# zhiqwang/demonet

Measured on AMD Instinct MI355X. Metric: images/sec ssdlite320_mobilenet_v3_large fp16 end-to-end incl. NMS, higher is better.
Workload: dtype fp16; 1 GPU; ssdlite320_mobilenet_v3_large fp16, batch 64 per GPU, 320x320 synthetic images, K=91, synthetic weights seed 0, post-process incl. per-class top-300 + hard NMS; global_batch=64, forwards_in_flight=3, parallelism=single GPU, input=NCHW fp32 in [0,1], device-resident

## Files before the change

### demonet_amd/_lib.py

```python
import ctypes as C
import os

_HERE = os.path.dirname(os.path.abspath(__file__))
LIB_PATH = os.environ.get("DEMONET_HIP_LIB") or os.path.join(_HERE, "lib", "libdemonet_hip.so")
DN_ABI_VERSION = 1

DN_OP = dict(stem=1, pw=2, dw=3, se=4, conv=5, maxpool=6, l2norm=7)
DN_T = dict(act=0, image=1, vec=2, pool=3)
DN_NMS = dict(hard=0, linear=1, gaussian=2)
DN_MERGE = dict(iou=0, ios=1)
DN_FRAME = dict(nv12=0, i420=1, rgb24=2, bgr24=3)
DN_COLOR = dict(bt601=0, bt709=1)
DN_COLOR_FULL_RANGE = 0x10
DN_REGION_HFLIP = 1
DN_SGD_CHUNK = 2048
DN_SGD_MAX_GATE = 8


class TensorDesc(C.Structure):
    _fields_ = [("c", C.c_int32), ("h", C.c_int32), ("w", C.c_int32), ("kind", C.c_int32)]


class OpDesc(C.Structure):
    _fields_ = [("type", C.c_int32), ("inp", C.c_int32), ("out", C.c_int32), ("residual", C.c_int32),
# ... 25 lines not shown

class TrackParams(C.Structure):
    _fields_ = [("track_thresh", C.c_float), ("low_thresh", C.c_float), ("new_thresh", C.c_float),
                ("match_thresh", C.c_float), ("second_thresh", C.c_float), ("unconfirmed_thresh", C.c_float),
                ("track_buffer", C.c_int32), ("class_agnostic", C.c_int32), ("max_tracks", C.c_int32), ("reserved", C.c_int32)]


class ModelDesc(C.Structure):
    _fields_ = [("abi_version", C.c_int32), ("n_tensors", C.c_int32), ("n_ops", C.c_int32),
                ("tensors", C.POINTER(TensorDesc)), ("ops", C.POINTER(OpDesc)),
                ("input_tensor", C.c_int32), ("image_h", C.c_int32), ("image_w", C.c_int32),
                ("mean", C.c_float * 3), ("std", C.c_float * 3),
                ("num_classes", C.c_int32), ("n_levels", C.c_int32),
                ("level_tensor", C.c_int32 * 8), ("anchors_per_loc", C.c_int32 * 8),
                ("num_anchors", C.c_int32), ("anchors", C.POINTER(C.c_float)),
                ("score_thresh", C.c_float), ("nms_thresh", C.c_float),
                ("detections_per_img", C.c_int32), ("topk_candidates", C.c_int32)]


_SIGNATURES = {
    "dn_abi_version": (C.c_int, []),
    "dn_last_error": (C.c_char_p, []),
    "dn_create": (C.c_int, [C.POINTER(ModelDesc), C.c_void_p, C.c_size_t, C.POINTER(C.c_void_p)]),
    "dn_destroy": (None, [C.c_void_p]),
    "dn_workspace_bytes": (C.c_size_t, [C.c_void_p, C.c_int]),
    "dn_forward": (C.c_int, [C.c_void_p, C.c_void_p, C.c_int, C.c_int, C.c_int, C.c_void_p, C.c_void_p, C.c_void_p,
                             C.c_void_p, C.c_void_p, C.c_size_t, C.c_void_p]),
    "dn_forward_u8": (C.c_int, [C.c_void_p, C.c_void_p, C.c_int, C.c_int, C.c_int, C.c_void_p, C.c_void_p, C.c_void_p,
                             C.c_void_p, C.c_void_p, C.c_size_t, C.c_void_p]),
    "dn_forward_frames": (C.c_int, [C.c_void_p, C.c_void_p, C.c_int, C.c_int, C.c_int, C.c_void_p, C.c_void_p, C.c_void_p,
                                    C.c_void_p, C.c_void_p, C.c_size_t, C.c_void_p]),
    "dn_forward_regions": (C.c_int, [C.c_void_p, C.c_void_p, C.c_void_p, C.c_int, C.c_int, C.c_int, C.c_void_p, C.c_void_p, C.c_void_p,
                                     C.c_void_p, C.c_void_p, C.c_size_t, C.c_void_p]),
    "dn_forward_heads": (C.c_int, [C.c_void_p, C.c_void_p, C.c_int, C.c_int, C.c_int, C.c_void_p, C.c_size_t, C.c_void_p]),
    "dn_head_outputs": (C.c_int, [C.c_void_p, C.c_void_p, C.c_int, C.POINTER(C.c_void_p), C.POINTER(C.c_void_p)]),
    "dn_tensor_ptr": (C.c_int, [C.c_void_p, C.c_void_p, C.c_int, C.c_int, C.POINTER(C.c_void_p), C.POINTER(C.c_size_t)]),
    "dn_postprocess_workspace_bytes": (C.c_size_t, [C.c_int, C.c_int, C.c_int, C.c_int, C.c_int]),
    "dn_postprocess": (C.c_int, [C.c_void_p, C.c_void_p, C.c_void_p, C.c_int, C.c_int, C.c_int, C.c_float, C.c_float,
                                 C.c_void_p, C.c_float, C.c_float, C.c_int, C.c_int, C.c_void_p, C.c_void_p, C.c_void_p,
                                 C.c_void_p, C.c_void_p, C.c_void_p, C.c_size_t, C.c_void_p]),
    "dn_postprocess_soft": (C.c_int, [C.c_void_p, C.c_void_p, C.c_void_p, C.c_int, C.c_int, C.c_int, C.c_float, C.c_float,
                                      C.c_void_p, C.c_float, C.c_float, C.c_int, C.c_float, C.c_int, C.c_int, C.c_void_p, C.c_void_p, C.c_void_p,
                                      C.c_void_p, C.c_void_p, C.c_void_p, C.c_size_t, C.c_void_p]),
    "dn_set_nms": (C.c_int, [C.c_void_p, C.c_int, C.c_float]),
    "dn_pointwise_conv": (C.c_int, [C.c_void_p, C.c_void_p, C.c_void_p, C.c_void_p, C.c_void_p, C.c_void_p, C.c_void_p, C.c_int,
                                    C.c_int, C.c_int, C.c_int, C.c_int, C.c_int, C.c_int64, C.c_void_p]),
    "dn_depthwise_conv": (C.c_int, [C.c_void_p, C.c_void_p, C.c_void_p, C.c_void_p, C.c_int, C.c_int, C.c_int, C.c_int,
                                    C.c_int, C.c_int, C.c_int, C.c_int, C.c_void_p]),
    "dn_depthwise_pool_blocks": (C.c_int, [C.c_int] * 6),
    "dn_depthwise_conv_pool": (C.c_int, [C.c_void_p] * 4 + [C.c_int] * 8 + [C.c_void_p] * 7 + [C.c_int, C.c_void_p]),
    "dn_dense_conv": (C.c_int, [C.c_void_p] * 5 + [C.c_int] * 10 + [C.c_void_p]),
    "dn_expand_depthwise": (C.c_int, [C.c_void_p] * 9 + [C.c_int] * 11 + [C.c_void_p]),
    "dn_expand_depthwise_tiles": (C.c_int, [C.c_int, C.c_int, C.c_int]),
    "dn_ssd_loss_workspace_bytes": (C.c_size_t, [C.c_int, C.c_int]),
    "dn_ssd_loss": (C.c_int, [C.c_void_p] * 6 + [C.c_int] * 4 + [C.c_float, C.c_float] + [C.c_void_p, C.c_void_p, C.c_void_p, C.c_size_t, C.c_void_p]),
    "dn_ssd_loss_state_bytes": (C.c_size_t, [C.c_int, C.c_int]),
    "dn_ssd_loss_train": (C.c_int, [C.c_void_p] * 6 + [C.c_int] * 4 + [C.c_float, C.c_float] + [C.c_void_p, C.c_void_p, C.c_void_p, C.c_size_t, C.c_void_p, C.c_size_t,
                                    C.c_void_p]),
    "dn_ssd_loss_backward": (C.c_int, [C.c_void_p] * 6 + [C.c_size_t, C.c_void_p] + [C.c_int] * 4 + [C.c_void_p] * 3),
    "dn_set_graph_mode": (C.c_int, [C.c_void_p, C.c_int]),
    "dn_set_packed_output": (C.c_int, [C.c_void_p, C.c_void_p]),
    "dn_profile_begin": (C.c_int, [C.c_void_p]),
    "dn_profile_end": (C.c_int, [C.c_void_p, C.POINTER(C.c_float), C.c_int]),
    "dn_batch_split": (C.c_int, [C.c_void_p, C.c_int]),
    "dn_set_chains": (C.c_int, [C.c_void_p, C.c_int]),
    "dn_profile_op_info": (C.c_int, [C.c_void_p, C.c_int, C.c_char_p, C.c_int, C.POINTER(C.c_int32)]),
    "dn_level_features": (C.c_int, [C.c_void_p, C.c_void_p, C.c_int, C.c_int, C.c_int, C.POINTER(C.c_void_p), C.POINTER(C.c_int), C.POINTER(C.c_int)]),
    "dn_forward_features": (C.c_int, [C.c_void_p, C.c_void_p, C.c_int, C.c_int, C.c_int, C.c_void_p, C.c_size_t, C.c_void_p]),
    "dn_lite_head_backward_workspace_bytes": (C.c_size_t, [C.c_int] * 6),
    "dn_lite_head_backward": (C.c_int, [C.c_void_p] * 5 + [C.c_int64] + [C.c_int] * 5 + [C.c_void_p] * 5 + [C.c_size_t, C.c_void_p]),
    "dn_crop_tiles": (C.c_int, [C.c_void_p, C.c_int, C.c_int, C.c_void_p, C.c_int, C.c_int, C.c_int, C.c_void_p, C.c_void_p]),
    "dn_merge_detections_workspace_bytes": (C.c_size_t, [C.c_int] * 3),
    "dn_merge_detections": (C.c_int, [C.c_void_p] * 5 + [C.c_int, C.c_int, C.POINTER(C.c_int32), C.c_int, C.c_int, C.c_float, C.c_int, C.c_int] + [C.c_void_p] * 6
                            + [C.c_size_t, C.c_void_p]),
    "dn_fuse_detections_workspace_bytes": (C.c_size_t, [C.c_int, C.c_int, C.POINTER(C.c_int32), C.c_int]),
    "dn_fuse_detections": (C.c_int, [C.c_void_p] * 6 + [C.c_int, C.c_int, C.POINTER(C.c_int32), C.c_int, C.c_float, C.c_float, C.c_int] + [C.c_void_p] * 6
                           + [C.c_size_t, C.c_void_p]),
    "dn_match_detections": (C.c_int, [C.c_void_p] * 8 + [C.c_int] * 4 + [C.POINTER(C.c_double), C.c_int, C.c_double] + [C.c_void_p] * 5),
    "dn_coco_match": (C.c_int, [C.c_void_p] * 9 + [C.c_int] * 4 + [C.POINTER(C.c_double), C.c_int, C.POINTER(C.c_double), C.c_int, C.c_int] + [C.c_void_p] * 5),
    "dn_augment_workspace_bytes": (C.c_size_t, [C.c_int]),
    "dn_augment_batch": (C.c_int, [C.POINTER(C.c_void_p), C.POINTER(C.c_int32), C.POINTER(C.c_int32), C.c_int, C.c_int, C.c_int, C.c_void_p, C.c_void_p, C.c_size_t, C.c_void_p]),
    "dn_sgd_workspace_bytes": (C.c_size_t, [C.c_int, C.c_int]),
    "dn_grad_norm": (C.c_int, [C.c_void_p, C.c_int, C.c_int, C.c_void_p, C.c_size_t, C.c_void_p, C.c_void_p]),
    "dn_sgd_step": (C.c_int, [C.c_void_p, C.c_int, C.c_int, SgdHyper, C.c_void_p, C.c_int, C.c_void_p, C.c_float, C.c_void_p, C.c_void_p]),
    "dn_track_state_bytes": (C.c_size_t, [C.c_int, C.c_int]),
    "dn_track_reset": (C.c_int, [C.c_void_p, C.c_int, C.c_int, C.c_void_p, C.c_void_p]),
    "dn_track_update": (C.c_int, [C.c_void_p] * 4 + [C.c_int, C.c_int, C.POINTER(TrackParams), C.c_void_p, C.c_size_t] + [C.c_void_p] * 8),
}
EXPORTS = tuple(_SIGNATURES)
_DEBUG_SIGNATURES = {
    "dn_debug_last_kernel": (C.c_int, [C.c_char_p, C.c_int]),
    "dn_debug_conv_pool": (C.c_int, [C.c_void_p] * 6 + [C.c_int] * 6 + [C.c_void_p]),
    "dn_debug_stem": (C.c_int, [C.c_void_p] * 4 + [C.c_int] * 7 + [C.POINTER(C.c_float), C.POINTER(C.c_float), C.c_int, C.c_int, C.c_void_p]),
    "dn_debug_choice": (C.c_int, [C.c_char_p, C.POINTER(C.c_int64), C.c_int, C.c_char_p, C.c_int]),
}

_lib = None


class HipLibraryMissing(RuntimeError):
    pass


def lib():
    global _lib
    if _lib is not None:
# ... 39 lines not shown
```

### demonet_amd/csrc/plan.hip

```cpp
#include <stdarg.h>
#include <stdlib.h>
#include <string.h>

#include <algorithm>
#include <cmath>
#include <atomic>
#include <map>
#include <mutex>
#include <set>
#include <string>
#include <tuple>
#include <vector>

#include "choice.h"

static thread_local char g_err[512] = "";

static thread_local char g_kernel[96] = "";
void dn_note_kernel(const char* fmt, ...) {
    va_list ap;
    va_start(ap, fmt);
    vsnprintf(g_kernel, sizeof(g_kernel), fmt, ap);
    va_end(ap);
}
// ... 1389 lines not shown
    a.nms_method = nms_method; a.nms_sigma = nms_sigma;
    a.boxes = boxes; a.scores = scores; a.labels = labels; a.counts = counts; a.kept_anchor = kept_anchor;
    a.ws = ws; a.ws_bytes = ws_bytes;
    a.xq = xcd_images_per_group(n);
    return launch_postprocess(a, reinterpret_cast<hipStream_t>(stream), nullptr);
}

extern "C" int dn_postprocess(const float* logits, const float* reg, const float* anchors, int n, int A, int K, float image_h,
                              float image_w, const float* scale_xy, float score_thresh, float nms_thresh, int topk, int dets,
                              float* boxes, float* scores, int64_t* labels, int32_t* counts, int32_t* kept_anchor, void* ws,
                              size_t ws_bytes, void* stream) {
    return dn_postprocess_soft(logits, reg, anchors, n, A, K, image_h, image_w, scale_xy, score_thresh, nms_thresh, DN_NMS_HARD, 0.f, topk, dets,
                               boxes, scores, labels, counts, kept_anchor, ws, ws_bytes, stream);
}

extern "C" int dn_pointwise_conv(const void* x, const void* w, const void* w_frag, const float* bias, const void* residual,
                                 const float* se, void* out, int m, int cin, int cout, int hw, int act, int out_fp32,
                                 int64_t out_img_stride, void* stream) {
    DN_REQUIRE(x && w && bias && out, "dn_pointwise_conv: null argument");
    PwArgs a;
    a.x = reinterpret_cast<const half_t*>(x); a.w = reinterpret_cast<const half_t*>(w); a.bias = bias;
    a.wfrag = reinterpret_cast<const half_t*>(w_frag);
    a.residual = reinterpret_cast<const half_t*>(residual); a.se = se; a.out = out;
    a.m = m; a.cin = cin; a.cout = cout; a.hw = hw; a.act = act; a.out_fp32 = out_fp32;
    a.out_img_stride = out_fp32 ? (long)out_img_stride : 0; a.out_base = 0;
    a.xq = (hw > 0 && m % hw == 0) ? xcd_images_per_group(m / hw) : 0;
    int rc = launch_pointwise(a, reinterpret_cast<hipStream_t>(stream));
    if (rc) return rc;
    DN_HIP_CHECK(hipGetLastError());
    return DN_OK;
}

extern "C" int dn_expand_depthwise(const void* x, const void* w1, const float* b1, const void* wd, const float* bd, const void* w3,
                                   const float* b3, void* out, float* pool_partial, int n, int h, int w, int cin, int cexp, int cout,
                                   int k, int stride, int act1, int act2, int has_res, void* stream) {
    DN_REQUIRE(x && wd && bd && out, "dn_expand_depthwise: null argument");
    DN_REQUIRE((w1 == nullptr) == (b1 == nullptr) && (w3 == nullptr) == (b3 == nullptr), "dn_expand_depthwise: weight without bias");
    ExpDwArgs a{};
    a.x = reinterpret_cast<const half_t*>(x); a.out = reinterpret_cast<half_t*>(out); a.pool = pool_partial;
    a.w1 = reinterpret_cast<const half_t*>(w1); a.b1 = b1; a.wd = reinterpret_cast<const half_t*>(wd); a.bd = bd;
    a.w3 = reinterpret_cast<const half_t*>(w3); a.b3 = b3;
    a.n = n; a.H = h; a.W = w; a.k = k; a.stride = stride; a.pad = (k - 1) / 2;
    a.Ho = (h + 2 * a.pad - k) / stride + 1; a.Wo = (w + 2 * a.pad - k) / stride + 1;
    a.cin = cin; a.cexp = cexp; a.cout = w3 ? cout : cexp; a.act1 = act1; a.act2 = act2; a.has_res = has_res;
    a.xq = xcd_images_per_group(n);
    int rc = launch_expdw(a, reinterpret_cast<hipStream_t>(stream));
    if (rc) return rc;
    DN_HIP_CHECK(hipGetLastError());
    return DN_OK;
}

extern "C" int dn_expand_depthwise_tiles(int ho, int wo, int stride) { return expdw_tiles_per_image(ho, wo, stride); }

extern "C" int dn_dense_conv(const void* x, const void* w, const float* bias, const void* zeros, void* out, int n, int h, int wd,
                             int cin, int cout, int k, int stride, int pad, int dil, int act, void* stream) {
    DN_REQUIRE(x && w && bias && out, "dn_dense_conv: null argument");
    DN_REQUIRE(n > 0 && h > 0 && wd > 0 && k >= 1 && stride >= 1 && dil >= 1 && pad >= 0, "dn_dense_conv: bad geometry");
    ConvArgs a;
    a.x = reinterpret_cast<const half_t*>(x); a.w = reinterpret_cast<const half_t*>(w); a.bias = bias; a.out = out;
    a.zeros = reinterpret_cast<const half_t*>(zeros);
    a.n = n; a.h = h; a.w_ = wd; a.cin = cin; a.cout = cout; a.k = k; a.stride = stride; a.pad = pad; a.dil = dil; a.act = act;
    a.ho = (h + 2 * pad - dil * (k - 1) - 1) / stride + 1;
    a.wo = (wd + 2 * pad - dil * (k - 1) - 1) / stride + 1;
    DN_REQUIRE(a.ho > 0 && a.wo > 0, "dn_dense_conv: empty output");
    a.out_fp32 = 0; a.out_img_stride = 0; a.out_base = 0;
    a.xq = xcd_images_per_group(n);
    int rc = launch_conv(a, reinterpret_cast<hipStream_t>(stream));
    if (rc) return rc;
    DN_HIP_CHECK(hipGetLastError());
    return DN_OK;
}

extern "C" int dn_depthwise_conv(const void* x, const void* w, const float* bias, void* out, int n, int h, int wd, int c, int k,
                                 int stride, int pad, int act, void* stream) {
    DN_REQUIRE(x && w && bias && out, "dn_depthwise_conv: null argument");
    DwArgs a;
    a.x = reinterpret_cast<const half_t*>(x); a.w = reinterpret_cast<const half_t*>(w); a.bias = bias;
    a.out = reinterpret_cast<half_t*>(out);
    a.n = n; a.h = h; a.w_ = wd; a.c = c; a.k = k; a.stride = stride; a.pad = pad; a.act = act;
    a.ho = (h + 2 * pad - k) / stride + 1;
    a.wo = (wd + 2 * pad - k) / stride + 1;
    a.xq = xcd_images_per_group(n);
    int rc = launch_depthwise(a, reinterpret_cast<hipStream_t>(stream));
    if (rc) return rc;
    DN_HIP_CHECK(hipGetLastError());
    return DN_OK;
}

extern "C" int dn_depthwise_pool_blocks(int h, int wd, int c, int k, int stride, int pad) {
    DwArgs a{};
    a.n = 1; a.h = h; a.w_ = wd; a.c = c; a.k = k; a.stride = stride; a.pad = pad;
    a.ho = (h + 2 * pad - k) / stride + 1;
    a.wo = (wd + 2 * pad - k) / stride + 1;
    return depthwise_pool_blocks(a);
}

extern "C" int dn_depthwise_conv_pool(const void* x, const void* w, const float* bias, void* out, int n, int h, int wd, int c, int k,
                                      int stride, int pad, int act, float* pool, const void* se_w1t, const float* se_b1, const void* se_w2t,
                                      const float* se_b2, float* se_scale, unsigned* se_counter, int squeeze, void* stream) {
    DN_REQUIRE(x && w && bias && out && pool, "dn_depthwise_conv_pool: null argument");
    DN_REQUIRE(!se_scale || (se_w1t && se_b1 && se_w2t && se_b2 && se_counter), "dn_depthwise_conv_pool: the squeeze-excitation tail needs both FCs and the counters");
    DwArgs a;
    a.x = reinterpret_cast<const half_t*>(x); a.w = reinterpret_cast<const half_t*>(w); a.bias = bias;
    a.out = reinterpret_cast<half_t*>(out);
    a.n = n; a.h = h; a.w_ = wd; a.c = c; a.k = k; a.stride = stride; a.pad = pad; a.act = act;
    a.ho = (h + 2 * pad - k) / stride + 1;
// ... 187 lines not shown
```

### demonet_amd/csrc/pwdirect.hip

```cpp
#include <algorithm>

#include "common.h"
#include "choice.h"

__device__ const uint4 g_pwdw_zero16 = {0u, 0u, 0u, 0u};

namespace {

typedef unsigned uint2v __attribute__((ext_vector_type(2)));

__device__ __forceinline__ void act16(floatx16& v, int act) {
    asm volatile("s_nop 7\n\ts_nop 3" : "+v"(v));
    if (act == DN_ACT_RELU) {
#pragma unroll
        for (int e = 0; e < 16; ++e) v[e] = dn_relu(v[e]);
    } else if (act == DN_ACT_RELU6) {
#pragma unroll
        for (int e = 0; e < 16; ++e) v[e] = dn_relu6(v[e]);
    } else if (act == DN_ACT_HSWISH) {
#pragma unroll
        for (int e = 0; e < 16; ++e) v[e] = v[e] * dn_relu6(v[e] + 3.f) * (1.f / 6.f);
    }
}

// ... 352 lines not shown
#pragma unroll
        for (int t = 0; t < 9; ++t) {
            const cp4 wp = (cp4)(q.wd + t * K + ks * 16);
            const u4v w0 = wp[0], w1 = wp[1];
            const uint4 wsel = make_uint4(hh ? w1[0] : w0[0], hh ? w1[1] : w0[1], hh ? w1[2] : w0[2], hh ? w1[3] : w0[3]);
            fma_mix_h8(acc, *reinterpret_cast<const uint4*>(&xin[t]), wsel);
        }
        dn_act_n<float[8], 8>(acc, q.act_dw);
#pragma unroll
        for (int e = 0; e < 8; ++e) xf[ks][e] = (half_t)acc[e];
    }
    const half8 zero8 = {0, 0, 0, 0, 0, 0, 0, 0};
    const half8 ones = {(half_t)1.f, (half_t)1.f, 0, 0, 0, 0, 0, 0};
    const half_t bhi = (half_t)bl;
    const half8 bw = {bhi, (half_t)(bl - (float)bhi), 0, 0, 0, 0, 0, 0};
    const bool bcol = kb == K;
    floatx16 acc;
#pragma unroll
    for (int e = 0; e < 16; ++e) acc[e] = 0.f;
#pragma unroll
    for (int ks = 0; ks < KSF; ++ks) acc = __builtin_amdgcn_mfma_f32_32x32x16_f16(wf[ks], xf[ks], acc, 0, 0, 0);
    acc = __builtin_amdgcn_mfma_f32_32x32x16_f16(bcol ? bw : zero8, bcol ? ones : zero8, acc, 0, 0, 0);
    act16(acc, a.act);
    if (has_res) {
#pragma unroll
        for (int g = 0; g < 4; ++g) {
            const half4 rr = __builtin_bit_cast(half4, rres[g]);
#pragma unroll
            for (int e = 0; e < 4; ++e) acc[4 * g + e] += (float)rr[e];
        }
    }
    uint2v p[4];
#pragma unroll
    for (int g = 0; g < 4; ++g) {
        half4 hv;
#pragma unroll
        for (int e = 0; e < 4; ++e) hv[e] = (half_t)acc[4 * g + e];
        p[g] = __builtin_bit_cast(uint2v, hv);
    }
    uint4 lo4, hi4;
    {
        const uint2v s0 = __builtin_amdgcn_permlane32_swap(p[0][0], p[1][0], false, false);
        const uint2v s1 = __builtin_amdgcn_permlane32_swap(p[0][1], p[1][1], false, false);
        const uint2v s2 = __builtin_amdgcn_permlane32_swap(p[2][0], p[3][0], false, false);
        const uint2v s3 = __builtin_amdgcn_permlane32_swap(p[2][1], p[3][1], false, false);
        lo4 = make_uint4(s0[0], s1[0], s0[1], s1[1]);
        hi4 = make_uint4(s2[0], s3[0], s2[1], s3[1]);
    }
    half_t* orow = reinterpret_cast<half_t*>(a.out) + (size_t)row * NC + hh * 8;
    const int c0 = hh * 8;
    if (row < mend) {
        if (c0 < NC) *reinterpret_cast<uint4*>(orow) = lo4;
        if (c0 + 16 < NC) *reinterpret_cast<uint4*>(orow + 16) = hi4;
    }
}


__device__ __forceinline__ void pw_glds16(const void* gsrc, unsigned dst) {
    unsigned keep;
    asm volatile("s_mov_b32 %0, m0\n\ts_mov_b32 m0, %2\n\ts_nop 0\n\tglobal_load_lds_dwordx4 %1, off\n\ts_mov_b32 m0, %0"
                 : "=&s"(keep) : "v"(gsrc), "s"(dst) : "memory");
}

template <int KS1, int RT>
__global__ __launch_bounds__(256) void pw_wstat_kernel(PwArgs a, int runs, int wg_per_group) {
    extern __shared__ __attribute__((aligned(16))) unsigned char pws_lds[];
    constexpr int KSF = KS1 - 1;
    typedef unsigned u32x4 __attribute__((ext_vector_type(4)));
    const int lane = threadIdx.x & 63, r = lane & 31, hh = lane >> 5;
    const int wave = __builtin_amdgcn_readfirstlane(threadIdx.x >> 6);
    const int K = a.cin, NC = a.cout;
    const int ksw = (K + 15) >> 4;
    int r0, mend, w;
    if (a.xq > 0) {
        const int g = blockIdx.x & 7;
        w = blockIdx.x >> 3;
        r0 = g * a.xq * a.hw;
        mend = min(a.m, r0 + a.xq * a.hw);
    } else {
        w = blockIdx.x; r0 = 0; mend = a.m;
    }
    const int run = w % runs, wgq = w / runs;
    const int Q = (wg_per_group / runs) * 4;
    const int n_units = mend > r0 ? (mend - r0 + 31) >> 5 : 0;
    const int ctiles = (NC + 31) >> 5;
    const int ct0 = run * RT;
    const unsigned lds0 = (unsigned)(size_t)(__attribute__((address_space(3))) unsigned char*)pws_lds;
    const unsigned xoff = (unsigned)(RT * ksw * 1024 + wave * ksw * 1024);
    auto dma_x = [&](int u) {
        const long row0 = (long)r0 + (long)u * 32;
        const unsigned char* src = reinterpret_cast<const unsigned char*>(a.x + row0 * K);
        const unsigned lim = (unsigned)min((long)(a.m - row0) * K * 2 - 16, 0x7fffffffL);
#pragma unroll 1
        for (int p = 0; p < ksw; ++p) pw_glds16(src + min((unsigned)(p * 1024 + lane * 16), lim), lds0 + xoff + p * 1024);
    };
    int u = wgq * 4 + wave;
    if (u < n_units) dma_x(u);
    {
        const unsigned char* wsrc = reinterpret_cast<const unsigned char*>(a.wfrag) + (size_t)ct0 * ksw * 1024 + lane * 16;
        const int pieces = max(min(RT, ctiles - ct0), 0) * ksw;
#pragma unroll 1
        for (int p = wave; p < pieces; p += 4) pw_glds16(wsrc + (size_t)p * 1024, lds0 + p * 1024);
    }
    float bl[RT];
#pragma unroll
    for (int t = 0; t < RT; ++t) bl[t] = a.bias[min((ct0 + t) * 32 + r, NC - 1)];
// ... 47 lines not shown
            }
            const uint2v s0 = __builtin_amdgcn_permlane32_swap(p[0][0], p[1][0], false, false);
            const uint2v s1 = __builtin_amdgcn_permlane32_swap(p[0][1], p[1][1], false, false);
            const uint2v s2 = __builtin_amdgcn_permlane32_swap(p[2][0], p[3][0], false, false);
            const uint2v s3 = __builtin_amdgcn_permlane32_swap(p[2][1], p[3][1], false, false);
            const uint2v q0 = __builtin_amdgcn_permlane16_swap(s0[0], s2[0], false, false);
            const uint2v q1 = __builtin_amdgcn_permlane16_swap(s1[0], s3[0], false, false);
            const uint2v q2 = __builtin_amdgcn_permlane16_swap(s0[1], s2[1], false, false);
            const uint2v q3 = __builtin_amdgcn_permlane16_swap(s1[1], s3[1], false, false);
            const u32x4 lo4 = {q0[0], q1[0], q2[0], q3[0]}, hi4 = {q0[1], q1[1], q2[1], q3[1]};
            const int col = (ct0 + t) * 32 + colq;
            const unsigned off = ((unsigned)rr * (unsigned)NC + (unsigned)col) * 2u;
            const bool okc = col < NC;
            __builtin_amdgcn_raw_buffer_store_b128(lo4, ors, (okc && rr < mend) ? off : 0x80000000u, 0, 0);
            __builtin_amdgcn_raw_buffer_store_b128(hi4, ors, (okc && rr + 16 < mend) ? off + 32u * (unsigned)NC : 0x80000000u, 0, 0);
        }
        asm volatile("s_waitcnt vmcnt(%0)" :: "n"(2 * RT) : "memory");
    }
}

template <int KS1, int RT>
int launch_wstat_t(const PwArgs& a, hipStream_t s) {
    const int ctiles = dn_cdiv(a.cout, 32), runs = dn_cdiv(ctiles, RT);
    const int groups = a.xq > 0 ? 8 : 1;
    const long rows = a.xq > 0 ? (long)a.xq * a.hw : a.m;
    const int units = dn_cdiv(rows, 32);
    int wpg = std::min(512 / groups, dn_cdiv(units, 4) * runs);
    wpg = std::max(runs, wpg / runs * runs);
    const int ksw = dn_cdiv(a.cin, 16);
    const int lds = (RT + 4) * ksw * 1024;
    dn_note_kernel("pw_wstat_kernel<%d,%d>", KS1, RT);
    hipLaunchKernelGGL((pw_wstat_kernel<KS1, RT>), dim3((unsigned)(groups * wpg)), dim3(256), lds, s, a, runs, wpg);
    return DN_OK;
}

template <int KSF, int TC>
int launch_t(const PwArgs& a, int wc_log, hipStream_t s) {
    const int BP = 32 * (4 >> wc_log), BC = (32 * TC) << wc_log;
    const int tiles = a.xq > 0 ? dn_cdiv((long)a.xq * a.hw, BP) : dn_cdiv(a.m, BP);
    const dim3 grid((unsigned)(a.xq > 0 ? 8 * tiles : tiles) * dn_cdiv(a.cout, BC));
    dn_note_kernel("pw_direct_kernel<%d,%d>", KSF, TC);
    hipLaunchKernelGGL((pw_direct_kernel<KSF, TC>), grid, dim3(256), 0, s, a, tiles, wc_log);
    return DN_OK;
}

}

bool pw_dw_direct_supported(const PwArgs& a, const DwArgs& d) {
    return dn_knob("DN_PW_DW", 1) != 0 && pw_direct_supported(a) && !a.se && (a.cin == 16 || a.cin == 32) && a.cout <= 32 && d.c == a.cin && d.k == 3 &&
           d.stride == 1 && d.pad == 1 && !d.pool && d.ho == d.h && d.wo == d.w_ && a.hw == d.h * d.w_ && (!a.residual || (a.residual == d.x && a.cout == a.cin)) &&
           a.hw >= 32 && fd_ok((unsigned long long)a.hw, (unsigned)d.w_);
}

int launch_pw_dw_direct(const PwArgs& a, const DwArgs& d, hipStream_t s) {
    DN_REQUIRE(pw_dw_direct_supported(a, d), "depthwise + pointwise (direct): unsupported cin=%d cout=%d", a.cin, a.cout);
    PwDwArgs q{};
    q.pw = a;
    q.pw.x = d.x;
    q.wd = d.w; q.bd = d.bias; q.h = d.h; q.w = d.w_; q.act_dw = d.act;
    q.inv_hw = 1.0f / (float)a.hw; q.fd_w = fastdiv((unsigned)d.w_);
    const int tiles = a.xq > 0 ? dn_cdiv((long)a.xq * a.hw, 128) : dn_cdiv(a.m, 128);
    const dim3 grid((unsigned)(a.xq > 0 ? 8 * tiles : tiles));
    dn_note_kernel("pw_dw_direct_kernel<%d>", a.cin / 16);
    if (a.cin == 16) hipLaunchKernelGGL((pw_dw_direct_kernel<1>), grid, dim3(256), 0, s, q, tiles);
    else hipLaunchKernelGGL((pw_dw_direct_kernel<2>), grid, dim3(256), 0, s, q, tiles);
    return DN_OK;
}

int launch_pw_direct(const PwArgs& a, const PwChoice& c, hipStream_t s) {
    const int ctiles = dn_cdiv(a.cout, 32);
    if (c.kernel == PwChoice::PW_WSTAT) {
        switch (c.k * 10 + c.t) {
#define DN_PWS_CASE(k, t) case k * 10 + t: return launch_wstat_t<k, t>(a, s);
            DN_PWS_CASE(2, 2) DN_PWS_CASE(2, 3) DN_PWS_CASE(2, 4) DN_PWS_CASE(3, 2) DN_PWS_CASE(3, 3) DN_PWS_CASE(3, 4) DN_PWS_CASE(4, 2) DN_PWS_CASE(4, 3) DN_PWS_CASE(4, 4)
            DN_PWS_CASE(5, 2) DN_PWS_CASE(5, 3) DN_PWS_CASE(5, 4) DN_PWS_CASE(6, 2) DN_PWS_CASE(6, 3) DN_PWS_CASE(6, 4) DN_PWS_CASE(7, 2) DN_PWS_CASE(7, 3)
            DN_PWS_CASE(8, 2) DN_PWS_CASE(8, 3) DN_PWS_CASE(9, 2)
#undef DN_PWS_CASE
        }
    } else if (c.kernel == PwChoice::PW_STREAM) {
        const long ptiles = dn_cdiv(a.m, 32 * c.t);
        int runs = (int)std::max(1L, std::min((long)ctiles, (long)2800 / ptiles));
        const int per = dn_cdiv(ctiles, runs);
        runs = dn_cdiv(ctiles, per);
        switch (c.k * 10 + c.t) {
            case 42: return launch_stream_t<4, 2>(a, runs, per, s);
            case 52: return launch_stream_t<5, 2>(a, runs, per, s);
            case 62: return launch_stream_t<6, 2>(a, runs, per, s);
            case 72: return launch_stream_t<7, 2>(a, runs, per, s);
            case 82: return launch_stream_t<8, 2>(a, runs, per, s);
        }
    } else if (c.kernel == PwChoice::PW_DIRECT && c.t == 2) {
        const int wc_log = ctiles <= 2 ? 0 : ctiles <= 4 ? 1 : 2;
        switch (c.k) {
#define DN_PWD_CASE2(k) case k: return launch_t<k, 2>(a, wc_log, s);
            DN_PWD_CASE2(0) DN_PWD_CASE2(1) DN_PWD_CASE2(2) DN_PWD_CASE2(3) DN_PWD_CASE2(4) DN_PWD_CASE2(5) DN_PWD_CASE2(6) DN_PWD_CASE2(7) DN_PWD_CASE2(8)
#undef DN_PWD_CASE2
        }
    } else if (c.kernel == PwChoice::PW_DIRECT) {
        const int wc_log = ctiles <= 1 ? 0 : ctiles <= 2 ? 1 : 2;
        switch (c.k) {
#define DN_PWD_CASE(k) case k: return launch_t<k, 1>(a, wc_log, s);
            DN_PWD_CASE(0) DN_PWD_CASE(1) DN_PWD_CASE(2) DN_PWD_CASE(3) DN_PWD_CASE(4) DN_PWD_CASE(5) DN_PWD_CASE(6) DN_PWD_CASE(7) DN_PWD_CASE(8)
            DN_PWD_CASE(9) DN_PWD_CASE(10) DN_PWD_CASE(11) DN_PWD_CASE(12) DN_PWD_CASE(13) DN_PWD_CASE(14) DN_PWD_CASE(15) DN_PWD_CASE(16)
#undef DN_PWD_CASE
        }
    }
    dn_set_error("pointwise (direct): no instantiation %d,%d for cin=%d cout=%d", c.k, c.t, a.cin, a.cout);
    return DN_E_UNSUPPORTED;
}
```

### include/demonet_hip.h

```cpp
#ifndef DEMONET_HIP_H
#define DEMONET_HIP_H

#include <stddef.h>
#include <stdint.h>

#ifdef __cplusplus
extern "C" {
#endif

#define DN_ABI_VERSION 1
#define DN_MAX_CLASSES 2048
#define DN_API __attribute__((visibility("default")))

enum { DN_OK = 0, DN_E_INVALID = -1, DN_E_HIP = -2, DN_E_WORKSPACE = -3, DN_E_UNSUPPORTED = -4 };

enum { DN_ACT_NONE = 0, DN_ACT_RELU = 1, DN_ACT_RELU6 = 2, DN_ACT_HSWISH = 3 };

enum { DN_OP_STEM = 1, DN_OP_PW = 2, DN_OP_DW = 3, DN_OP_SE = 4, DN_OP_CONV = 5, DN_OP_MAXPOOL = 6, DN_OP_L2NORM = 7 };

enum { DN_T_ACT = 0, DN_T_IMAGE = 1, DN_T_VEC = 2, DN_T_POOL = 3 };

typedef struct dn_tensor_desc {
    int32_t c, h, w, kind;
} dn_tensor_desc;
// ... 64 lines not shown
    int32_t frame;
    int32_t x0, y0, width, height;
    int32_t flags;
    int32_t reserved[2];
} dn_region;
DN_API int dn_forward_regions(dn_plan* plan, const dn_frame* frames_dev, const dn_region* regions_dev, int n, int format, int color,
                       float* boxes_dev, float* scores_dev, int64_t* labels_dev, int32_t* counts_dev,
                       void* workspace_dev, size_t workspace_bytes, void* stream);

DN_API int dn_forward_heads(dn_plan* plan, const float* images_dev, int n, int h, int w,
                     void* workspace_dev, size_t workspace_bytes, void* stream);
DN_API int dn_head_outputs(const dn_plan* plan, void* workspace_dev, int n, float** cls_logits_dev, float** bbox_regression_dev);
DN_API int dn_tensor_ptr(const dn_plan* plan, void* workspace_dev, int n, int tensor_id, void** ptr, size_t* bytes);

DN_API int dn_level_features(const dn_plan* plan, void* workspace_dev, int n, int level, int chain, void** ptr, int* first_image, int* images);
DN_API int dn_forward_features(dn_plan* plan, const float* images_dev, int n, int h, int w,
                               void* workspace_dev, size_t workspace_bytes, void* stream);

DN_API size_t dn_postprocess_workspace_bytes(int n, int num_anchors, int num_classes, int topk_candidates, int detections_per_img);
DN_API int dn_postprocess(const float* cls_logits_dev, const float* bbox_regression_dev, const float* anchors_dev,
                   int n, int num_anchors, int num_classes,
                   float image_h, float image_w, const float* scale_xy_dev ,
                   float score_thresh, float nms_thresh, int topk_candidates, int detections_per_img,
                   float* boxes_dev, float* scores_dev, int64_t* labels_dev, int32_t* counts_dev,
                   int32_t* kept_anchor_dev, void* workspace_dev, size_t workspace_bytes, void* stream);

enum { DN_NMS_HARD = 0, DN_NMS_SOFT_LINEAR = 1, DN_NMS_SOFT_GAUSSIAN = 2 };
DN_API int dn_set_nms(dn_plan* plan, int method, float sigma);
DN_API int dn_postprocess_soft(const float* cls_logits_dev, const float* bbox_regression_dev, const float* anchors_dev,
                   int n, int num_anchors, int num_classes,
                   float image_h, float image_w, const float* scale_xy_dev ,
                   float score_thresh, float nms_thresh, int nms_method, float nms_sigma, int topk_candidates, int detections_per_img,
                   float* boxes_dev, float* scores_dev, int64_t* labels_dev, int32_t* counts_dev,
                   int32_t* kept_anchor_dev, void* workspace_dev, size_t workspace_bytes, void* stream);

DN_API int dn_pointwise_conv(const void* x_dev, const void* w_dev, const void* w_frag_dev, const float* bias_dev,
                      const void* residual_dev, const float* se_scale_dev, void* out_dev, int m, int cin, int cout, int hw,
                      int act, int out_fp32, int64_t out_img_stride, void* stream);
DN_API int dn_dense_conv(const void* x_dev, const void* w_dev, const float* bias_dev, const void* zeros_dev, void* out_dev,
                  int n, int h, int w, int cin, int cout, int k, int stride, int pad, int dil, int act, void* stream);
DN_API int dn_depthwise_conv(const void* x_dev, const void* w_dev, const float* bias_dev, void* out_dev,
                      int n, int h, int w, int c, int k, int stride, int pad, int act, void* stream);
DN_API int dn_depthwise_pool_blocks(int h, int w, int c, int k, int stride, int pad);
DN_API int dn_depthwise_conv_pool(const void* x_dev, const void* w_dev, const float* bias_dev, void* out_dev,
                      int n, int h, int w, int c, int k, int stride, int pad, int act, float* pool_dev,
                      const void* se_w1t_dev, const float* se_b1_dev, const void* se_w2t_dev, const float* se_b2_dev,
                      float* se_scale_dev, unsigned* se_counter_dev, int squeeze, void* stream);

DN_API int dn_expand_depthwise(const void* x_dev, const void* w1_dev, const float* b1_dev, const void* wd_dev, const float* bd_dev,
                        const void* w3_dev, const float* b3_dev, void* out_dev, float* pool_partial_dev,
                        int n, int h, int w, int cin, int cexp, int cout, int k, int stride, int act1, int act2, int has_res,
                        void* stream);
DN_API int dn_expand_depthwise_tiles(int ho, int wo, int stride);

DN_API int dn_set_graph_mode(dn_plan* plan, int enabled);

DN_API int dn_profile_begin(dn_plan* plan);
DN_API int dn_profile_end(dn_plan* plan, float* ms_per_op , int capacity);
DN_API int dn_profile_op_info(const dn_plan* plan, int op_index, char* kernel, int capacity, int32_t* owner);

DN_API int dn_set_packed_output(dn_plan* plan, float* packed_dev);

DN_API int dn_batch_split(const dn_plan* plan, int n);
DN_API int dn_set_chains(dn_plan* plan, int chains);

DN_API size_t dn_ssd_loss_workspace_bytes(int n, int num_anchors);
DN_API int dn_ssd_loss(const float* cls_logits_dev, const float* bbox_regression_dev, const float* anchors_dev,
                       const float* gt_boxes_dev, const int64_t* gt_labels_dev, const int32_t* gt_counts_dev,
                       int n, int num_anchors, int num_classes, int gmax, float iou_thresh, float neg_to_pos_ratio,
                       int64_t* matched_idxs_dev, float* losses_dev, void* workspace_dev, size_t workspace_bytes, void* stream);

DN_API size_t dn_ssd_loss_state_bytes(int n, int num_anchors);
DN_API int dn_ssd_loss_train(const float* cls_logits_dev, const float* bbox_regression_dev, const float* anchors_dev,
                             const float* gt_boxes_dev, const int64_t* gt_labels_dev, const int32_t* gt_counts_dev,
                             int n, int num_anchors, int num_classes, int gmax, float iou_thresh, float neg_to_pos_ratio,
                             int64_t* matched_idxs_dev, float* losses_dev, void* workspace_dev, size_t workspace_bytes,
                             void* state_dev, size_t state_bytes, void* stream);
DN_API int dn_ssd_loss_backward(const float* cls_logits_dev, const float* bbox_regression_dev, const float* anchors_dev,
                                const float* gt_boxes_dev, const int64_t* gt_labels_dev, const void* state_dev, size_t state_bytes,
                                const float* grad_losses_dev, int n, int num_anchors, int num_classes, int gmax,
                                float* grad_cls_logits_dev, float* grad_bbox_regression_dev, void* stream);

DN_API size_t dn_lite_head_backward_workspace_bytes(int n, int h, int w, int c, int cout, int depthwise);
DN_API int dn_lite_head_backward(const void* x_dev, const void* wd_dev, const float* bd_dev, const void* w1_dev, const float* dy_dev,
                                 int64_t dy_img_stride, int n, int h, int w, int c, int cout, float* g_wd_dev, float* g_bd_dev,
                                 float* g_w1_dev, float* g_b1_dev, void* workspace_dev, size_t workspace_bytes, void* stream);

DN_API int dn_crop_tiles(const float* image_dev, int h, int w, const int32_t* origins_dev, int t, int th, int tw, float* out_dev, void* stream);

enum { DN_MERGE_IOU = 0, DN_MERGE_IOS = 1 };
DN_API size_t dn_merge_detections_workspace_bytes(int s_total, int d, int groups);
DN_API int dn_merge_detections(const float* boxes_dev, const float* scores_dev, const int64_t* labels_dev, const int32_t* counts_dev,
                               const float* offsets_dev, int s_total, int d, const int32_t* group_begin, int groups, int metric, float thresh,
                               int class_agnostic, int d_out, float* boxes_out_dev, float* scores_out_dev, int64_t* labels_out_dev,
                               int32_t* counts_out_dev, int32_t* src_out_dev, void* workspace_dev, size_t workspace_bytes, void* stream);

DN_API size_t dn_fuse_detections_workspace_bytes(int s_total, int d, const int32_t* group_begin, int groups);
DN_API int dn_fuse_detections(const float* boxes_dev, const float* scores_dev, const int64_t* labels_dev, const int32_t* counts_dev,
                              const float* offsets_dev, const float* weights_dev, int s_total, int d, const int32_t* group_begin, int groups,
                              float thresh, float skip_thresh, int d_out, float* boxes_out_dev, float* scores_out_dev, int64_t* labels_out_dev,
                              int32_t* counts_out_dev, int32_t* members_out_dev, void* workspace_dev, size_t workspace_bytes, void* stream);

DN_API int dn_match_detections(const float* boxes_dev, const float* scores_dev, const int64_t* labels_dev, const int32_t* counts_dev,
                               const float* gt_boxes_dev, const int64_t* gt_labels_dev, const uint8_t* gt_difficult_dev,
                               const int32_t* gt_counts_dev, int n, int d, int gmax, int num_classes, const double* thresholds, int n_thresh,
                               double pixel_offset, uint32_t* flags_dev, int32_t* best_gt_dev, double* best_ov_dev, int64_t* gt_stats_dev,
// ... 63 lines not shown
```

Baseline: 110,400 images/sec.

## Stage depthwise input band with halo in LDS for fused dw+pw kernel

Adds an LDS-staged variant of the fused depthwise 3x3 plus pointwise kernel. Each block loads a band of pixel rows plus a halo into shared memory with an XOR swizzle, then computes the 9 taps from LDS instead of re-reading global memory for each tap. The new path is enabled by default, and a standalone dn_depthwise_pointwise entry point is exposed. This trades added LDS footprint, occupancy limits and redundant halo loads for less global traffic. The layer only handles cin of 16 or 32.

```diff
diff --git a/demonet_amd/_lib.py b/demonet_amd/_lib.py
--- a/demonet_amd/_lib.py
+++ b/demonet_amd/_lib.py
@@ -101,6 +101,7 @@
     "dn_dense_conv": (C.c_int, [C.c_void_p] * 5 + [C.c_int] * 10 + [C.c_void_p]),
     "dn_expand_depthwise": (C.c_int, [C.c_void_p] * 9 + [C.c_int] * 11 + [C.c_void_p]),
     "dn_expand_depthwise_tiles": (C.c_int, [C.c_int, C.c_int, C.c_int]),
+    "dn_depthwise_pointwise": (C.c_int, [C.c_void_p] * 6 + [C.c_int] * 8 + [C.c_void_p]),
     "dn_ssd_loss_workspace_bytes": (C.c_size_t, [C.c_int, C.c_int]),
     "dn_ssd_loss": (C.c_int, [C.c_void_p] * 6 + [C.c_int] * 4 + [C.c_float, C.c_float] + [C.c_void_p, C.c_void_p, C.c_void_p, C.c_size_t, C.c_void_p]),
     "dn_ssd_loss_state_bytes": (C.c_size_t, [C.c_int, C.c_int]),
diff --git a/demonet_amd/csrc/plan.hip b/demonet_amd/csrc/plan.hip
--- a/demonet_amd/csrc/plan.hip
+++ b/demonet_amd/csrc/plan.hip
@@ -1465,6 +1465,31 @@
 
 extern "C" int dn_expand_depthwise_tiles(int ho, int wo, int stride) { return expdw_tiles_per_image(ho, wo, stride); }
 
+extern "C" int dn_depthwise_pointwise(const void* x, const void* wd, const float* bd, const void* w, const float* b, void* out, int n, int h,
+                                      int wdt, int c, int cout, int act_dw, int act, int has_res, void* stream) {
+    DN_REQUIRE(x && wd && bd && w && b && out, "dn_depthwise_pointwise: null argument");
+    DN_REQUIRE(n > 0 && h > 0 && wdt > 0 && c > 0 && cout > 0, "dn_depthwise_pointwise: bad geometry");
+    if (!dn_rows_fit(n, (long)h * wdt)) {
+        dn_set_error("dn_depthwise_pointwise: n=%d images of %d x %d pixels do not fit 32-bit row indices", n, h, wdt);
+        return DN_E_UNSUPPORTED;
+    }
+    DwArgs d{};
+    d.x = reinterpret_cast<const half_t*>(x); d.w = reinterpret_cast<const half_t*>(wd); d.bias = bd;
+    d.n = n; d.h = h; d.w_ = wdt; d.c = c; d.k = 3; d.stride = 1; d.pad = 1; d.act = act_dw; d.ho = h; d.wo = wdt;
+    PwArgs a{};
+    a.x = d.x; a.w = reinterpret_cast<const half_t*>(w); a.bias = b; a.residual = has_res ? d.x : nullptr; a.se = nullptr; a.out = out;
+    a.m = n * h * wdt; a.cin = c; a.cout = cout; a.hw = h * wdt; a.act = act; a.out_fp32 = 0; a.out_img_stride = 0; a.out_base = 0;
+    a.xq = d.xq = xcd_images_per_group(n);
+    if (!pw_dw_direct_supported(a, d)) {
+        dn_set_error("dn_depthwise_pointwise: unsupported n=%d h=%d w=%d c=%d cout=%d has_res=%d", n, h, wdt, c, cout, has_res);
+        return DN_E_UNSUPPORTED;
+    }
+    int rc = launch_pw_dw_direct(a, d, reinterpret_cast<hipStream_t>(stream));
+    if (rc) return rc;
+    DN_HIP_CHECK(hipGetLastError());
+    return DN_OK;
+}
+
 extern "C" int dn_dense_conv(const void* x, const void* w, const float* bias, const void* zeros, void* out, int n, int h, int wd,
                              int cin, int cout, int k, int stride, int pad, int dil, int act, void* stream) {
     DN_REQUIRE(x && w && bias && out, "dn_dense_conv: null argument");
diff --git a/demonet_amd/csrc/pwdirect.hip b/demonet_amd/csrc/pwdirect.hip
--- a/demonet_amd/csrc/pwdirect.hip
+++ b/demonet_amd/csrc/pwdirect.hip
@@ -428,6 +428,168 @@
     if (row < mend) {
         if (c0 < NC) *reinterpret_cast<uint4*>(orow) = lo4;
         if (c0 + 16 < NC) *reinterpret_cast<uint4*>(orow + 16) = hi4;
+    }
+}
+
+constexpr int PW_DW_LDS_MAX = 64 * 1024;
+
+__device__ __forceinline__ void fma_mix_h8_from(float (&acc)[8], const float (&c)[8], const uint4& e, const uint4& w) {
+    const unsigned ee[4] = {e.x, e.y, e.z, e.w}, ww[4] = {w.x, w.y, w.z, w.w};
+#pragma unroll
+    for (int i = 0; i < 4; ++i) {
+        asm volatile("v_fma_mix_f32 %0, %1, %2, %3 op_sel_hi:[1,1,0]" : "=v"(acc[2 * i]) : "v"(ee[i]), "v"(ww[i]), "v"(c[2 * i]));
+        asm volatile("v_fma_mix_f32 %0, %1, %2, %3 op_sel:[1,1,0] op_sel_hi:[1,1,0]" : "=v"(acc[2 * i + 1]) : "v"(ee[i]), "v"(ww[i]), "v"(c[2 * i + 1]));
+    }
+}
+
+template <int KSF>
+__global__ __launch_bounds__(256, KSF == 1 ? 4 : 2) void pw_dw_direct_lds_kernel(PwDwArgs q, int n, int bands, int band, int halo) {
+    extern __shared__ __attribute__((aligned(16))) unsigned char pdl_lds[];
+    constexpr int PB = 32 * KSF;
+    constexpr unsigned SWM = 2 * KSF - 1;
+    typedef unsigned u32x4 __attribute__((ext_vector_type(4)));
+    const PwArgs& a = q.pw;
+    const int lane = threadIdx.x & 63, r = lane & 31, hh = lane >> 5;
+    const int wave = __builtin_amdgcn_readfirstlane(threadIdx.x >> 6);
+    constexpr int K = 16 * KSF;
+    const int NC = a.cout;
+    int img, bi;
+    if (!xcd_image_of(blockIdx.x, bands, a.xq, n, img, bi)) return;
+    const int b0 = bi * band, blen = min(band, a.hw - b0);
+    const int nslots = blen + 2 * halo;
+    const unsigned zoff = (unsigned)nslots * PB;
+    {
+        const __amdgpu_buffer_rsrc_t xrs =
+            __builtin_amdgcn_make_buffer_rsrc(const_cast<half_t*>(a.x + (size_t)img * a.hw * K), 0, a.hw * PB, 0x00020000);
+        const int chunks = nslots * (2 * KSF);
+        const unsigned g0 = (unsigned)((b0 - halo) * PB);
+        for (int c0 = threadIdx.x; c0 < chunks; c0 += 8 * 256) {
+            u32x4 v[8];
+#pragma unroll
+            for (int i = 0; i < 8; ++i) {
+                const int c = c0 + i * 256;
+                v[i] = __builtin_amdgcn_raw_buffer_load_b128(xrs, c < chunks ? g0 + (unsigned)c * 16u : 0x80000000u, 0, 0);
+            }
+            asm volatile("" : "+v"(v[0]), "+v"(v[1]), "+v"(v[2]), "+v"(v[3]), "+v"(v[4]), "+v"(v[5]), "+v"(v[6]), "+v"(v[7]));
+#pragma unroll
+            for (int i = 0; i < 8; ++i) {
+                const unsigned A = (unsigned)(c0 + i * 256) * 16u;
+                if (c0 + i * 256 < chunks) *reinterpret_cast<u32x4*>(pdl_lds + (A ^ (((A >> 8) & SWM) << 4))) = v[i];
+            }
+        }
+        if (threadIdx.x < 4) *reinterpret_cast<u32x4*>(pdl_lds + zoff + threadIdx.x * 16) = u32x4{0u, 0u, 0u, 0u};
+    }
+    const int nrow = min(r, NC - 1);
+    const half_t* wpt = a.w + (size_t)nrow * K + hh * 8;
+    half8 wf[KSF];
+#pragma unroll
+    for (int ks = 0; ks < KSF; ++ks) wf[ks] = *reinterpret_cast<const half8*>(wpt + ks * 16);
+    const float bl = a.bias[nrow];
+    typedef unsigned u4v __attribute__((ext_vector_type(4)));
+    typedef float f4v __attribute__((ext_vector_type(4)));
+    typedef const __attribute__((address_space(4))) u4v* cp4;
+    typedef const __attribute__((address_space(4))) f4v* cpf4;
+    uint4 wsel[KSF][9];
+    float bsel[KSF][8];
+#pragma unroll
+    for (int ks = 0; ks < KSF; ++ks) {
+        const cpf4 bp = (cpf4)(q.bd + ks * 16);
+        const f4v c0 = bp[0], c1 = bp[1], c2 = bp[2], c3 = bp[3];
+#pragma unroll
+        for (int e = 0; e < 4; ++e) { bsel[ks][e] = hh ? c2[e] : c0[e]; bsel[ks][4 + e] = hh ? c3[e] : c1[e]; }
+#pragma unroll
+        for (int t = 0; t < 9; ++t) {
+            const cp4 wp = (cp4)(q.wd + t * K + ks * 16);
+            const u4v w0 = wp[0], w1 = wp[1];
+            wsel[ks][t] = make_uint4(hh ? w1[0] : w0[0], hh ? w1[1] : w0[1], hh ? w1[2] : w0[2], hh ? w1[3] : w0[3]);
+        }
+    }
+    const half8 zero8 = {0, 0, 0, 0, 0, 0, 0, 0};
+    const half8 ones = {(half_t)1.f, (half_t)1.f, 0, 0, 0, 0, 0, 0};
+    const half_t bhi = (half_t)bl;
+    const half8 bw = {bhi, (half_t)(bl - (float)bhi), 0, 0, 0, 0, 0, 0};
+    const bool bcol = hh == 0;
+    const half8 wlast = bcol ? bw : zero8, xlast = bcol ? ones : zero8;
+    const bool has_res = a.residual != nullptr;
+    int toff[9], roff;
+    {
+        const int s0 = wave * 32 + r + halo;
+#pragma unroll
+        for (int t = 0; t < 9; ++t) {
+            const int d = (t / 3 - 1) * q.w + (t % 3 - 1);
+            const unsigned sw = (((unsigned)(s0 + d) * PB >> 8) & SWM) << 4;
+            toff[t] = d * PB + (int)((unsigned)(hh * 16) ^ sw);
+        }
+        roff = (int)((((unsigned)s0 * PB >> 8) & SWM) << 4);
+    }
+    __syncthreads();
+    half_t* const obase = reinterpret_cast<half_t*>(a.out) + ((size_t)img * a.hw + b0) * NC + hh * 8;
+    const int ntiles = (blen + 31) >> 5;
+    for (int t = wave; t < ntiles; t += 4) {
+        const int pl = t * 32 + r, plc = min(pl, blen - 1);
+        const unsigned p = (unsigned)(b0 + plc);
+        const int px = (int)(p - fd_div(p, q.fd_w) * (unsigned)q.w);
+        const bool okl = px > 0, okr = px < q.w - 1;
+        const unsigned S = (unsigned)(plc + halo) * PB;
+        unsigned ad[9];
+#pragma unroll
+        for (int tp = 0; tp < 9; ++tp) {
+            const unsigned A = S + (unsigned)toff[tp];
+            ad[tp] = (tp % 3 == 0) ? (okl ? A : zoff) : (tp % 3 == 2) ? (okr ? A : zoff) : A;
+        }
+        half8 xf[KSF];
+#pragma unroll
+        for (int ks = 0; ks < KSF; ++ks) {
+            half8 xin[9];
+#pragma unroll
+            for (int tp = 0; tp < 9; ++tp) xin[tp] = *reinterpret_cast<const half8*>(pdl_lds + (ad[tp] ^ (unsigned)(ks * 32)));
+            float acc[8];
+            fma_mix_h8_from(acc, bsel[ks], *reinterpret_cast<const uint4*>(&xin[0]), wsel[ks][0]);
+#pragma unroll
+            for (int tp = 1; tp < 9; ++tp) fma_mix_h8(acc, *reinterpret_cast<const uint4*>(&xin[tp]), wsel[ks][tp]);
+            dn_act_n<float[8], 8>(acc, q.act_dw);
+#pragma unroll
+            for (int e = 0; e < 8; ++e) xf[ks][e] = (half_t)acc[e];
+        }
+        uint2 rres[2 * KSF];
+        if (has_res) {
+#pragma unroll
+            for (int g = 0; g < 2 * KSF; ++g) rres[g] = *reinterpret_cast<const uint2*>(pdl_lds + S + ((unsigned)(g * 16) ^ (unsigned)roff) + hh * 8);
+        }
+        floatx16 acc;
+#pragma unroll
+        for (int e = 0; e < 16; ++e) acc[e] = 0.f;
+#pragma unroll
+        for (int ks = 0; ks < KSF; ++ks) acc = __builtin_amdgcn_mfma_f32_32x32x16_f16(wf[ks], xf[ks], acc, 0, 0, 0);
+        acc = __builtin_amdgcn_mfma_f32_32x32x16_f16(wlast, xlast, acc, 0, 0, 0);
+        act16(acc, a.act);
+        if (has_res) {
+#pragma unroll
+            for (int g = 0; g < 2 * KSF; ++g) {
+                const half4 rr = __builtin_bit_cast(half4, rres[g]);
+#pragma unroll
+                for (int e = 0; e < 4; ++e) acc[4 * g + e] += (float)rr[e];
+            }
+        }
+        uint2v pk[4];
+#pragma unroll
+        for (int g = 0; g < 4; ++g) {
+            half4 hv;
+#pragma unroll
+            for (int e = 0; e < 4; ++e) hv[e] = (half_t)acc[4 * g + e];
+            pk[g] = __builtin_bit_cast(uint2v, hv);
+        }
+        const uint2v s0 = __builtin_amdgcn_permlane32_swap(pk[0][0], pk[1][0], false, false);
+        const uint2v s1 = __builtin_amdgcn_permlane32_swap(pk[0][1], pk[1][1], false, false);
+        const uint2v s2 = __builtin_amdgcn_permlane32_swap(pk[2][0], pk[3][0], false, false);
+        const uint2v s3 = __builtin_amdgcn_permlane32_swap(pk[2][1], pk[3][1], false, false);
+        const uint4 lo4 = make_uint4(s0[0], s1[0], s0[1], s1[1]), hi4 = make_uint4(s2[0], s3[0], s2[1], s3[1]);
+        half_t* orow = obase + (size_t)pl * NC;
+        const int c0 = hh * 8;
+        if (pl < blen) {
+            if (c0 < NC) *reinterpret_cast<uint4*>(orow) = lo4;
+            if (c0 + 16 < NC) *reinterpret_cast<uint4*>(orow + 16) = hi4;
+        }
     }
 }
 
@@ -581,6 +743,17 @@
            a.hw >= 32 && fd_ok((unsigned long long)a.hw, (unsigned)d.w_);
 }
 
+struct PwDwLds { int band, halo, bands, lds; };
+static bool pw_dw_lds_geometry(const PwArgs& a, const DwArgs& d, PwDwLds& g) {
+    const int pb = a.cin * 2;
+    g.band = std::max(32, dn_knob("DN_PW_DW_BAND", DN_PW_DW_BAND) & ~31);
+    g.halo = (d.w_ + 1 + 3) & ~3;
+    g.bands = dn_cdiv(a.hw, g.band);
+    const long lds = ((long)std::min(g.band, a.hw) + 2L * g.halo) * pb + 64;
+    g.lds = (int)std::min(lds, (long)PW_DW_LDS_MAX + 1);
+    return lds <= PW_DW_LDS_MAX && (long)a.hw * pb < (1L << 31) && (long)(d.n + 7) * g.bands < (1L << 31);
+}
+
 int launch_pw_dw_direct(const PwArgs& a, const DwArgs& d, hipStream_t s) {
     DN_REQUIRE(pw_dw_direct_supported(a, d), "depthwise + pointwise (direct): unsupported cin=%d cout=%d", a.cin, a.cout);
     PwDwArgs q{};
@@ -588,9 +761,16 @@
     q.pw.x = d.x;
     q.wd = d.w; q.bd = d.bias; q.h = d.h; q.w = d.w_; q.act_dw = d.act;
     q.inv_hw = 1.0f / (float)a.hw; q.fd_w = fastdiv((unsigned)d.w_);
+    dn_note_kernel("pw_dw_direct_kernel<%d>", a.cin / 16);
+    PwDwLds g;
+    if (dn_knob("DN_PW_DW_LDS", 1) != 0 && a.m == (long)d.n * a.hw && pw_dw_lds_geometry(a, d, g)) {
+        const dim3 grid((unsigned)(a.xq > 0 ? 8 * a.xq : d.n) * g.bands);
+        if (a.cin == 16) hipLaunchKernelGGL((pw_dw_direct_lds_kernel<1>), grid, dim3(256), g.lds, s, q, d.n, g.bands, g.band, g.halo);
+        else hipLaunchKernelGGL((pw_dw_direct_lds_kernel<2>), grid, dim3(256), g.lds, s, q, d.n, g.bands, g.band, g.halo);
+        return DN_OK;
+    }
     const int tiles = a.xq > 0 ? dn_cdiv((long)a.xq * a.hw, 128) : dn_cdiv(a.m, 128);
     const dim3 grid((unsigned)(a.xq > 0 ? 8 * tiles : tiles));
-    dn_note_kernel("pw_dw_direct_kernel<%d>", a.cin / 16);
     if (a.cin == 16) hipLaunchKernelGGL((pw_dw_direct_kernel<1>), grid, dim3(256), 0, s, q, tiles);
     else hipLaunchKernelGGL((pw_dw_direct_kernel<2>), grid, dim3(256), 0, s, q, tiles);
     return DN_OK;
diff --git a/include/demonet_hip.h b/include/demonet_hip.h
--- a/include/demonet_hip.h
+++ b/include/demonet_hip.h
@@ -140,6 +140,10 @@
                         int n, int h, int w, int cin, int cexp, int cout, int k, int stride, int act1, int act2, int has_res,
                         void* stream);
 DN_API int dn_expand_depthwise_tiles(int ho, int wo, int stride);
+
+#define DN_PW_DW_BAND 640
+DN_API int dn_depthwise_pointwise(const void* x_dev, const void* wd_dev, const float* bd_dev, const void* w_dev, const float* b_dev,
+                           void* out_dev, int n, int h, int w, int c, int cout, int act_dw, int act, int has_res, void* stream);
 
 DN_API int dn_set_graph_mode(dn_plan* plan, int enabled);
 
```

New measurement: 114,100 images/sec (median of 6 runs). 1.03x the previous value.
